# tomcreutz/slam-uwv_kalman_filters

Measured on AMD Instinct MI355X. Metric: UKF predict+update steps/sec at batch=65536 PoseUKF instances, 1 & 8 GPU, higher is better.
Workload: dtype f64

## Files before the change

### slam-uwv_kalman_filters_amd/csrc/uwvk_dev.hpp

```cpp
#pragma once
#include <hip/hip_runtime.h>
#include <stdint.h>

#include <cmath>

#define UWVK_DEV __device__ __forceinline__

namespace uwvk {

void clear_hip_error();
void note_hip_error(int err, const char* where);
inline int edevice_status(hipError_t e, const char* where) {
  note_hip_error((int)e, where);
  return 5;
}
inline int launch_sync_status(hipError_t launch, hipStream_t st, const char* where) {
  const hipError_t s = hipStreamSynchronize(st);
  if (launch != hipSuccess) return edevice_status(launch, where);
  if (s != hipSuccess) return edevice_status(s, where);
  return 0;
}
struct DeviceGuard {
  int prev = -1;
  explicit DeviceGuard(int device) {
// ... 58 lines not shown
}

UWVK_DEV void qmul(const double a[4], const double b[4], double o[4]) {
  double w = a[0] * b[0] - a[1] * b[1] - a[2] * b[2] - a[3] * b[3];
  double x = a[0] * b[1] + a[1] * b[0] + a[2] * b[3] - a[3] * b[2];
  double y = a[0] * b[2] + a[2] * b[0] + a[3] * b[1] - a[1] * b[3];
  double z = a[0] * b[3] + a[3] * b[0] + a[1] * b[2] - a[2] * b[1];
  o[0] = w; o[1] = x; o[2] = y; o[3] = z;
}

UWVK_DEV void qrot(const double q[4], const double v[3], double o[3]) {
  double uv[3], t[3];
  cross3(q + 1, v, uv);
  uv[0] += uv[0]; uv[1] += uv[1]; uv[2] += uv[2];
  cross3(q + 1, uv, t);
#pragma unroll
  for (int i = 0; i < 3; i++) o[i] = v[i] + q[0] * uv[i] + t[i];
}
UWVK_DEV void qrot_inv(const double q[4], const double v[3], double o[3]) {
  double c[4] = {q[0], -q[1], -q[2], -q[3]};
  qrot(c, v, o);
}
UWVK_DEV void qmatrix(const double q[4], double R[9]) {
  double w = q[0], x = q[1], y = q[2], z = q[3];
  double tx = 2 * x, ty = 2 * y, tz = 2 * z;
  double twx = tx * w, twy = ty * w, twz = tz * w;
  double txx = tx * x, txy = ty * x, txz = tz * x;
  double tyy = ty * y, tyz = tz * y, tzz = tz * z;
  R[0] = 1 - (tyy + tzz); R[1] = txy - twz; R[2] = txz + twy;
  R[3] = txy + twz; R[4] = 1 - (txx + tzz); R[5] = tyz - twx;
  R[6] = txz - twy; R[7] = tyz + twx; R[8] = 1 - (txx + tyy);
}

UWVK_DEV void so3_exp(const double v[3], double o[4]) {
  double t = sqrt(v[0] * v[0] + v[1] * v[1] + v[2] * v[2]);
  if (t == 0.0) { o[0] = 1; o[1] = o[2] = o[3] = 0; return; }
  double s, c;
  sincos(0.5 * t, &s, &c);
  s = s / t;
  o[0] = c; o[1] = s * v[0]; o[2] = s * v[1]; o[3] = s * v[2];
}
UWVK_DEV void so3_log(const double q[4], double o[3]) {
  double w = q[0], x = q[1], y = q[2], z = q[3];
  if (w < 0) { w = -w; x = -x; y = -y; z = -z; }
  double nv = sqrt(x * x + y * y + z * z);
  if (nv == 0.0) { o[0] = o[1] = o[2] = 0; return; }
  double k = 2.0 * atan2(nv, w) / nv;
  o[0] = k * x; o[1] = k * y; o[2] = k * z;
}
UWVK_DEV void qboxminus(const double a[4], const double b[4], double o[3]) {
  double bc[4] = {b[0], -b[1], -b[2], -b[3]}, r[4];
  qmul(a, bc, r);
  so3_log(r, o);
}

UWVK_DEV void qmul_side(const double a[4], const double b[4], double o[4], int swap) {
  const double sg = swap ? -1.0 : 1.0;
  const double cx = a[2] * b[3] - a[3] * b[2], cy = a[3] * b[1] - a[1] * b[3], cz = a[1] * b[2] - a[2] * b[1];
  o[0] = a[0] * b[0] - a[1] * b[1] - a[2] * b[2] - a[3] * b[3];
  o[1] = a[0] * b[1] + a[1] * b[0] + sg * cx;
  o[2] = a[0] * b[2] + a[2] * b[0] + sg * cy;
  o[3] = a[0] * b[3] + a[3] * b[0] + sg * cz;
}
UWVK_DEV void qplus_side(const double e[4], const double q[4], double o[4], int right) {
  if (!right) {
    qmul(e, q, o);
    return;
  }
  qmul_side(e, q, o, 1);
}
UWVK_DEV void qboxminus_side(const double a[4], const double b[4], double o[3], int right) {
  double bc[4] = {b[0], -b[1], -b[2], -b[3]}, r[4];
  if (!right) {
    qmul(a, bc, r);
  } else {
    qmul_side(a, bc, r, 1);
  }
  so3_log(r, o);
}

UWVK_DEV int lane_id() { return threadIdx.x & 63; }

UWVK_DEV int64_t xcd_instance(int64_t batch) {
  const int64_t w = blockIdx.x, n = batch >> 3;
  return w < (n << 3) ? (w & 7) * n + (w >> 3) : w;
}

UWVK_DEV constexpr int pidx(int i, int j) { return i >= j ? i * (i + 1) / 2 + j : j * (j + 1) / 2 + i; }
template <int DOF>
constexpr int tri_n() { return DOF * (DOF + 1) / 2; }

UWVK_DEV void unpack(int e, int& i, int& j) {
  int r = (int)((__builtin_sqrtf(8.0f * (float)e + 1.0f) - 1.0f) * 0.5f);
  if ((r + 1) * (r + 2) / 2 <= e) r++;
  if (r * (r + 1) / 2 > e) r--;
  i = r;
  j = e - r * (r + 1) / 2;
}

UWVK_DEV double shfl_d(double v, int src) {
  int lo = __double2loint(v), hi = __double2hiint(v);
  lo = __shfl(lo, src, 64);
  hi = __shfl(hi, src, 64);
  return __hiloint2double(hi, lo);
}
UWVK_DEV double readlane_d(double v, int lane) {
  int lo = __builtin_amdgcn_readlane(__double2loint(v), lane);
  int hi = __builtin_amdgcn_readlane(__double2hiint(v), lane);
  return __hiloint2double(hi, lo);
}
UWVK_DEV double shfl_xor_d(double v, int m) {
  int lo = __double2loint(v), hi = __double2hiint(v);
  lo = __shfl_xor(lo, m, 64);
  hi = __shfl_xor(hi, m, 64);
  return __hiloint2double(hi, lo);
}
UWVK_DEV double wave_sum(double v) {
#pragma unroll
  for (int m = 32; m >= 1; m >>= 1) v += shfl_xor_d(v, m);
  return v;
}

typedef double d4_t __attribute__((ext_vector_type(4)));

UWVK_DEV d4_t mfma_f64(double a, double b, d4_t c) { return __builtin_amdgcn_mfma_f64_16x16x4f64(a, b, c, 0, 0, 0); }

#ifdef UWVK_STAMPS
static __device__ unsigned long long uwvk_stamp_sum[64];
static __device__ unsigned long long uwvk_stamp_cnt[64];
UWVK_DEV unsigned long long stamp_now() {
  unsigned long long t;
  asm volatile("s_memtime %0\n\ts_waitcnt lgkmcnt(0)" : "=s"(t)::"memory");
  return t;
}
struct Stamper {
  unsigned long long last;
  UWVK_DEV Stamper() : last(stamp_now()) {}
  UWVK_DEV void mark(int ph) {
    __builtin_amdgcn_sched_barrier(0);
    const unsigned long long t = stamp_now();
    __builtin_amdgcn_sched_barrier(0);
    if (threadIdx.x == 0 && (blockIdx.x & 63) == 0) {
      atomicAdd(&uwvk_stamp_sum[ph], t - last);
      atomicAdd(&uwvk_stamp_cnt[ph], 1ull);
    }
    last = t;
  }
};
#else
struct Stamper {
  UWVK_DEV void mark(int) {}
};
#endif
#define UWVK_STAMP(ph) \
  do {                 \
    if (st) st->mark(ph); \
  } while (0)

}
```

### slam-uwv_kalman_filters_amd/csrc/uwvk_psp_dev.hpp

```cpp
#pragma once
#include <cstddef>

#include "uwvk_pose_dev.hpp"


#ifndef PSP_PAIR
#define PSP_PAIR 0
#endif
#ifndef PSP_NS
#define PSP_NS psp
#endif

namespace uwvk {
namespace PSP_NS {

constexpr int kLanes = PSP_PAIR ? 32 : 64;

UWVK_DEV void chain_prio_hi() { __builtin_amdgcn_s_setprio(1); }
UWVK_DEV void chain_prio_lo() { __builtin_amdgcn_s_setprio(0); }

template <int DOF>
struct PG {
  static constexpr int NP = DOF * (DOF + 1) / 2;
  static constexpr int NSLOT = (NP + kLanes - 1) / kLanes;
  static constexpr int N = 2 * DOF + 1;
  static constexpr int KP = 15;
  static constexpr int STG = 115;
};

template <int DOF>
struct alignas(16) PspSmem {
  double S[PG<DOF>::NP];
  double mu[Lay<DOF>::store];
  double stg[PG<DOF>::STG];
};
static_assert(sizeof(PspSmem<53>) <= 12800, "12 instances per CU");
static_assert(offsetof(PspSmem<53>, mu) == sizeof(double) * PG<53>::NP, "mu follows S");
static_assert(offsetof(PspSmem<53>, stg) == sizeof(double) * (PG<53>::NP + Lay<53>::store), "stg follows mu");
static_assert(offsetof(PspSmem<26>, mu) == sizeof(double) * PG<26>::NP, "mu follows S");
static_assert(offsetof(PspSmem<26>, stg) == sizeof(double) * (PG<26>::NP + Lay<26>::store), "stg follows mu");
constexpr int kPdLane0 = 27, kPdN = 27;
template <int DOF>
struct alignas(16) PspSmemPD : PspSmem<DOF> {
  double pS[32];
  double pm[32];
};
template <int DOF, int PD>
struct SmemT {
  using type = PspSmem<DOF>;
};
template <int DOF>
struct SmemT<DOF, 1> {
  using type = PspSmemPD<DOF>;
};
template <int DOF>
UWVK_DEV double* pd_ptr(PspSmem<DOF>&) {
  return nullptr;
}
template <int DOF>
UWVK_DEV double* pd_ptr(PspSmemPD<DOF>& s) {
  return s.pS;
}
UWVK_DEV constexpr int pd_dof(int d) { return d < 19 ? d : d + 27; }
UWVK_DEV constexpr int pd_store(int s) { return s < 20 ? s : s + 27; }

template <int DOF>
UWVK_DEV double* flat(PspSmem<DOF>& sm) {
  return reinterpret_cast<double*>(&sm);
}
template <int DOF>
UWVK_DEV const double* flat(const PspSmem<DOF>& sm) {
  return reinterpret_cast<const double*>(&sm);
}
template <int DOF>
constexpr int kFlatMu = PG<DOF>::NP;


UWVK_DEV int olane() {
  int l = PSP_PAIR ? ((int)threadIdx.x & 31) : (int)threadIdx.x;
  asm volatile("" : "+v"(l));
  return l;
}

template <class F>
UWVK_DEV constexpr unsigned long long lane_mask(F f) {
  unsigned long long m = 0;
  for (int i = 0; i < 64; i++)
    if (f(PSP_PAIR ? (i & 31) : i)) m |= 1ull << i;
  return m;
}
UWVK_DEV constexpr unsigned long long rep_mask(unsigned long long m) {
  return PSP_PAIR ? ((m & 0xFFFFFFFFull) | ((m & 0xFFFFFFFFull) << 32)) : m;
}
UWVK_DEV constexpr bool mask_needs_split(unsigned long long m) {
  return m >= 0xFFFFFFFF80000000ull && m < 0xFFFFFFFFFFFFFFF0ull;
}
UWVK_DEV bool lane_in_split(unsigned long long m) {
  unsigned lo = (unsigned)m, hi = (unsigned)(m >> 32);
  asm volatile("" : "+s"(lo), "+s"(hi));
  return __builtin_amdgcn_inverse_ballot_w64(((unsigned long long)hi << 32) | lo);
}
template <unsigned long long M>
UWVK_DEV bool lane_const() {
  if constexpr (mask_needs_split(M)) return lane_in_split(M);
  else return __builtin_amdgcn_inverse_ballot_w64(M);
}
#define LANE_IF(l, expr)                                                                                        \
  ({                                                                                                            \
    constexpr unsigned long long m_ = ::uwvk::PSP_NS::lane_mask([](int l) constexpr { return (bool)(expr); }); \
    ::uwvk::PSP_NS::lane_const<m_>();                                                                           \
  })
#define LANE_IN(m)                                                                     \
  (::uwvk::PSP_NS::mask_needs_split(::uwvk::PSP_NS::rep_mask(m))                       \
       ? ::uwvk::PSP_NS::lane_in_split(::uwvk::PSP_NS::rep_mask(m))                    \
       : __builtin_amdgcn_inverse_ballot_w64(::uwvk::PSP_NS::rep_mask(m)))
UWVK_DEV bool upper_half() { return lane_const<0xFFFFFFFF00000000ull>(); }
#if PSP_PAIR
template <int J>
UWVK_DEV double hbc(double v) {
  static_assert(J >= 0 && J < 16, "row_newbcast lane");
  int lo = __builtin_amdgcn_mov_dpp(__double2loint(v), 0x150 + J, 0xf, 0xf, false);
  int hi = __builtin_amdgcn_mov_dpp(__double2hiint(v), 0x150 + J, 0xf, 0xf, false);
  lo = __builtin_amdgcn_update_dpp(lo, lo, 0x142, 0xa, 0xf, false);
  hi = __builtin_amdgcn_update_dpp(hi, hi, 0x142, 0xa, 0xf, false);
  return __hiloint2double(hi, lo);
}
#endif
UWVK_DEV double hread(double v, int j) {
#if PSP_PAIR
  if (__builtin_constant_p(j) && j >= 0 && j < 16) {
    switch (j) {
      case 0: return hbc<0>(v);
      case 1: return hbc<1>(v);
      case 2: return hbc<2>(v);
      case 3: return hbc<3>(v);
      case 4: return hbc<4>(v);
      case 5: return hbc<5>(v);
      case 6: return hbc<6>(v);
      case 7: return hbc<7>(v);
      case 8: return hbc<8>(v);
      case 9: return hbc<9>(v);
      case 10: return hbc<10>(v);
      case 11: return hbc<11>(v);
      case 12: return hbc<12>(v);
      case 13: return hbc<13>(v);
      case 14: return hbc<14>(v);
      default: return hbc<15>(v);
    }
  }
  const double a = readlane_d(v, j), b = readlane_d(v, 32 + j);
  return upper_half() ? b : a;
#else
  return readlane_d(v, j);
#endif
}
UWVK_DEV int hlane(int j) { return PSP_PAIR ? j + ((int)threadIdx.x & 32) : j; }
// ... 54 lines not shown
#if PSP_PAIR
  static_assert(NL <= 32, "pair: one instance per 32-lane half");
  if constexpr (NL <= 16) return hread(s, 15);
  s = s + dpp_d<0x142, 0xa, 0xf>(s);
  return hread(s, 31);
#else
  if constexpr (NL <= 16) return readlane_d(s, 15);
  s = s + dpp_d<0x142, 0xa, 0xf>(s);
  if constexpr (NL <= 32) return readlane_d(s, 31);
  s = s + dpp_d<0x143, 0xc, 0xf>(s);
  return readlane_d(s, 63);
#endif
}
UWVK_DEV double sk(double c) {
  asm volatile("" : "+s"(c));
  return c;
}
UWVK_DEV void so3_exp_psp(const double v[3], double o[4]) {
  const double t2 = v[0] * v[0] + v[1] * v[1] + v[2] * v[2];
  if (t2 < 0.0625) {
    const double u = 0.25 * t2;
    double s = u * sk(-1.0 / 39916800.0);
    s = s + sk(1.0 / 362880.0);
    s = fma(s, u, sk(-1.0 / 5040.0));
    s = fma(s, u, sk(1.0 / 120.0));
    s = fma(s, u, sk(-1.0 / 6.0));
    s = fma(s, u, 1.0);
    s = 0.5 * s;
    double c = u * sk(-1.0 / 3628800.0);
    c = c + sk(1.0 / 40320.0);
    c = fma(c, u, sk(-1.0 / 720.0));
    c = fma(c, u, sk(1.0 / 24.0));
    c = fma(c, u, -0.5);
    c = fma(c, u, 1.0);
    o[0] = c; o[1] = s * v[0]; o[2] = s * v[1]; o[3] = s * v[2];
  } else {
    so3_exp(v, o);
  }
}
UWVK_DEV void so3_log_psp(const double q[4], double o[3]) {
  double w = q[0], x = q[1], y = q[2], z = q[3];
  if (w < 0) { w = -w; x = -x; y = -y; z = -z; }
  const double n2 = x * x + y * y + z * z, w2 = w * w;
  if (n2 < 0.0025 * w2) {
    double iw = __builtin_amdgcn_rcp(w);
    iw = fma(iw, fma(-w, iw, 1.0), iw);
    iw = fma(iw, fma(-w, iw, 1.0), iw);
    const double r2 = n2 * (iw * iw);
    double a = r2 * sk(-1.0 / 13.0);
    a = fma(a, -r2, sk(1.0 / 11.0));
    a = fma(a, -r2, sk(1.0 / 9.0));
    a = fma(a, -r2, sk(1.0 / 7.0));
    a = fma(a, -r2, sk(1.0 / 5.0));
    a = fma(a, -r2, sk(1.0 / 3.0));
    a = fma(a, -r2, 1.0);
    const double k = 2.0 * a * iw;
    o[0] = k * x; o[1] = k * y; o[2] = k * z;
  } else {
    so3_log(q, o);
  }
}
template <int SR>
UWVK_DEV void qplus_psp(const double e[4], const double q[4], double o[4]) {
  if constexpr (SR) qmul(q, e, o);
  else qmul(e, q, o);
}
template <int SR>
UWVK_DEV void qboxminus_psp(const double a[4], const double b[4], double o[3]) {
  double bc[4] = {b[0], -b[1], -b[2], -b[3]}, r[4];
  if constexpr (SR) qmul(bc, a, r);
  else qmul(a, bc, r);
  so3_log_psp(r, o);
}

UWVK_DEV double swap_pair_d(double v) { return dpp_d<0xb1, 0xf, 0xf>(v); }

UWVK_DEV double sel3(double v0, double v1, double v2, int i) { return i == 0 ? v0 : (i == 1 ? v1 : v2); }
UWVK_DEV double sel6(double v0, double v1, double v2, double v3, double v4, double v5, int i) {
  return i < 3 ? sel3(v0, v1, v2, i) : sel3(v3, v4, v5, i - 3);
}

UWVK_DEV int pidx_sel(int p, int j, int Tj) { return j >= p ? Tj + p : p * (p + 1) / 2 + j; }
UWVK_DEV int pidx_sel_b(int p, int j, int Tj, bool ge) { return ge ? Tj + p : p * (p + 1) / 2 + j; }

UWVK_DEV void wsync() {
  __builtin_amdgcn_fence(__ATOMIC_RELEASE, "wavefront");
  __builtin_amdgcn_wave_barrier();
  __builtin_amdgcn_fence(__ATOMIC_ACQUIRE, "wavefront");
}

template <int R, int NL, int STRIDE>
UWVK_DEV void lds_sums(const double (&v)[R], double* buf, int l, double (&out)[R]) {
  static_assert(NL % 2 == 0 && R * NL <= 115, "transpose buffer (PG::STG)");
  const int c = l / STRIDE;
  if (l % STRIDE == 0 && c < NL) {
#pragma unroll
    for (int i = 0; i < R; i++) buf[i * NL + c] = v[i];
  }
  wsync();
  const double* row = buf + (l < R ? l : 0) * NL;
  double p[NL / 2];
#pragma unroll
  for (int k = 0; k < NL / 2; k++) p[k] = row[2 * k] + row[2 * k + 1];
#pragma unroll
  for (int w = 1; w < NL / 2; w *= 2)
#pragma unroll
    for (int k = 0; k + w < NL / 2; k += 2 * w) p[k] += p[k + w];
#pragma unroll
  for (int i = 0; i < R; i++) out[i] = hread(p[0], i);
}

#define PSP_PHASE(ph) \
  do {                \
    UWVK_STAMP(ph);   \
    l = olane();      \
  } while (0)

UWVK_DEV void psync() {
  __builtin_amdgcn_fence(__ATOMIC_RELEASE, "workgroup");
  __builtin_amdgcn_s_barrier();
  __builtin_amdgcn_fence(__ATOMIC_ACQUIRE, "workgroup");
}

UWVK_DEV constexpr bool scaled_dof(int d) { return d >= 12 && d != 18; }

template <int K, int J>
UWVK_DEV void pchol_step_lds(double (&a)[K], int r, bool& ok, double* col, double* rows, int q, double piv,
                             double inv_in, double& chk) {
  if constexpr (J < K) {
    ok = ok && (piv > 0.0);
    const double inv = rsqrt_f64(piv);
    a[J] = LANE_IF(r, r >= J) ? a[J] * inv : 0.0;
    double pnext = 0.0, invn = 0.0;
    if constexpr (J + 1 < K) {
      pnext = hread(a[J + 1] - a[J] * a[J], J + 1);
    }
    if constexpr (J + 1 < K) {
      constexpr int C0 = J + 1;
      double* const cj = col + (((C0 & 1) == 0) ? 1 : 0);
      static_assert(64 + 1 <= 115, "column slots (PG::STG)");
      cj[r & 63] = a[J];
      __builtin_amdgcn_fence(__ATOMIC_RELEASE, "wavefront");
      __builtin_amdgcn_wave_barrier();
      __builtin_amdgcn_fence(__ATOMIC_ACQUIRE, "wavefront");
#pragma unroll
      for (int c = C0; c < K; c++) a[c] -= a[J] * cj[c];
#pragma unroll
      for (int c = J + 1; c < K; c++) asm volatile("" : "+v"(a[c]));
    }
    pchol_step_lds<K, J + 1>(a, r, ok, col, rows, q, pnext, invn, chk);
  }
}

constexpr int STG_ROWS = 0;

template <int DOF, int K, class RL>
UWVK_DEV bool pchol(const double* S, int r, double (&a)[K], double dl, double* stg) {
  const int rr = r < DOF ? r : DOF - 1;
  const double* Sr = S + rr * (rr + 1) / 2;
#pragma unroll
  for (int c = 0; c < K; c++) a[c] = Sr[c] * (scaled_dof(c) ? dl * hread(dl, c) : dl);
  bool ok = true;
  static_assert(rows_ascending<RL>(), "RL::rows ascending");
  constexpr unsigned long long rm = rep_mask(rows_mask<RL>());
  int q = (int)__builtin_amdgcn_mbcnt_hi((unsigned)(rm >> 32), __builtin_amdgcn_mbcnt_lo((unsigned)rm, 0u));
  if constexpr (PSP_PAIR) q -= upper_half() ? __builtin_popcount((unsigned)rm) : 0;
  static_assert(RL::NR >= 1 && STG_ROWS + RL::NR * K <= 115, "staging area (PG::STG)");
  const double p0 = hread(a[0], 0);
  const double inv0 = rsqrt_f64(p0);
  double chk = fma(inv0, 0.0, 0.0);
  pchol_step_lds<K, 0>(a, r, ok, stg + STG_ROWS, stg + STG_ROWS, q, p0, inv0, chk);
  if (LANE_IN(rows_mask<RL>())) {
    double* rp = stg + STG_ROWS + q * K;
#pragma unroll
    for (int J = 0; J < K; J++) rp[J] = a[J];
  }
  psync();
  return ok;
}

template <int NR>
UWVK_DEV constexpr int row_pos(const int (&rows)[NR], int d) {
  for (int q = 0; q < NR; q++)
    if (rows[q] == d) return q;
  return -1;
}

template <class RL, int DOF, int K, int Q>
UWVK_DEV void gen_rows_q(const double* mu, const double* stg, int j, double sg, double (&v)[3], double* x) {
  if constexpr (Q < RL::NR) {
    constexpr int d = RL::rows[Q];
    const double l = stg[Q * K + j];
    if constexpr (d >= 3 && d < 6) {
      v[d - 3] = sg * l;
    } else {
      x[d2s(d)] = mu[d2s(d)] + sg * l;
    }
    gen_rows_q<RL, DOF, K, Q + 1>(mu, stg, j, sg, v, x);
  }
}
template <class RL>
UWVK_DEV constexpr bool has_rot() {
  for (int q = 0; q < RL::NR; q++)
    if (RL::rows[q] >= 3 && RL::rows[q] < 6) return true;
  return false;
}
template <class RL, int DOF, int K, int SR>
UWVK_DEV void gen_rows(const double* mu, const double* stg, int p, double x[Lay<DOF>::store]) {
  using L = Lay<DOF>;
#pragma unroll
  for (int s = 0; s < L::store; s++) x[s] = mu[s];
  if constexpr (K > 0) {
    const bool in = LANE_IF(p, p < 2 * K);
    const int j = in ? (p >> 1) : 0;
    const double sg = in ? (LANE_IF(p, (p & 1) != 0) ? -1.0 : 1.0) : 0.0;
    double v[3] = {0.0, 0.0, 0.0};
    gen_rows_q<RL, DOF, K, 0>(mu, stg, j, sg, v, x);
    if constexpr (has_rot<RL>()) {
      double e[4];
      so3_exp_psp(v, e);
      qplus_psp<SR>(e, mu + L::s_quat, x + L::s_quat);
    }
  }
}

template <int DOF, int SR>
UWVK_DEV void proc_orientation(const double x[Lay<DOF>::store], const PoseShared& sh, const ProcCtx& c, double o[4]) {
  using L = Lay<DOF>;
  const double dl = x[L::s_pos] * sh.inv_rm;
  double sl, cl;
  if (fabs(dl) < 0.01) {
    const double u = dl * dl;
    double sd = fma(fma(fma(u * sk(1.0 / 362880.0) + sk(-1.0 / 5040.0), u, sk(1.0 / 120.0)), u, sk(-1.0 / 6.0)), u, 1.0) * dl;
    double cd = fma(fma(fma(u * sk(1.0 / 40320.0) + sk(-1.0 / 720.0), u, sk(1.0 / 24.0)), u, -0.5), u, 1.0);
    sl = sh.slat0 * cd + sh.clat0 * sd;
    cl = sh.clat0 * cd - sh.slat0 * sd;
  } else {
    sincos(sh.lat0 + dl, &sl, &cl);
  }
  const double er[3] = {kEarthW * cl, 0.0, kEarthW * sl};
  double wb[3], wn[3];
#pragma unroll
  for (int i = 0; i < 3; i++) wb[i] = c.w[i] - x[L::s_bg + i];
  qrot(x + L::s_quat, wb, wn);
#pragma unroll
  for (int i = 0; i < 3; i++) wn[i] = (wn[i] - er[i]) * c.dt;
  double e[4];
  so3_exp_psp(wn, e);
  qplus_psp<SR>(e, x + L::s_quat, o);
}

UWVK_DEV double proc_vect_lane(int s, const double* mu, const ProcCtx& c) {
  const double x = mu[s];
  const double y = mu[c.vpart >= 0 ? c.vpart : s];
  const double d = c.vpart >= 0 ? y : c.nt_lane * (x - c.off_lane);
  return (c.vpart >= 0 || c.nt_lane != 0.0) ? x + c.dt * d : x;
}

template <int DOF>
UWVK_DEV double tan_ntau_sel(int d, const PoseShared& sh) {
  using L = Lay<DOF>;
  double nt = 0.0;
  nt = (d >= L::d_bg && d < L::d_bg + 3) ? sh.ntau[0] : nt;
  nt = (d >= L::d_ba && d < L::d_ba + 3) ? sh.ntau[1] : nt;
  if constexpr (L::has_params) {
    nt = (d >= L::d_inertia && d < L::d_inertia + 9) ? sh.ntau[2] : nt;
    nt = (d >= L::d_lin && d < L::d_lin + 9) ? sh.ntau[3] : nt;
    nt = (d >= L::d_quad && d < L::d_quad + 9) ? sh.ntau[4] : nt;
  }
  nt = (d >= L::d_wv && d < L::d_wv + 4) ? sh.ntau[5] : nt;
  nt = (d >= L::d_badcp && d < L::d_badcp + 2) ? sh.ntau[6] : nt;
  nt = (d == L::d_rho) ? sh.ntau[7] : nt;
  return nt;
}
UWVK_DEV constexpr int proc_couple(int d) { return d < 3 ? d + 6 : (d >= 6 && d < 9 ? d + 3 : -1); }

struct PredRows {
  static constexpr int NR = 7;
  static constexpr int rows[NR] = {0, 3, 4, 5, 12, 13, 14};
};

struct LaneQ {
  double q0, q1, q2;
};
template <int DOF, int PD = 0>
UWVK_DEV LaneQ lane_q(const double* fq, int l) {
  const double2* f2 = reinterpret_cast<const double2*>(fq);
  LaneQ q{0.0, 0.0, 0.0};
  if (l < DOF) {
    q.q0 = f2[pidx(l, l)].y;
    if (l >= 1) q.q1 = f2[pidx(l, l - 1)].y;
    if (l >= 2) q.q2 = f2[pidx(l, l - 2)].y;
  }
  if constexpr (PD && !PSP_PAIR) {
    if (l >= kPdLane0 && l < kPdLane0 + kPdN) q.q0 = f2[PG<DOF>::NP + (l - kPdLane0)].y;
  }
  return q;
}

template <int DOF, int QM = 0, int SR = 0, int PD = 0>
UWVK_DEV bool psp_predict(PspSmem<DOF>& sm, const PoseShared& sh, const ProcCtx& pc, const double* Q,
                          const double* fq, double& ds, double& ids, const LaneQ& lq,
                          Stamper* st = nullptr, double* px = nullptr) {
  using L = Lay<DOF>;
  using G = PG<DOF>;
  constexpr int K = G::KP;
  static_assert(!PD || (DOF == 26 && QM == 1), "PD: the 26-DOF layout, lane-resident Q");
  constexpr int NW = PD ? 53 : DOF;
  int l = olane();
  const double dt = pc.dt, dt2 = dt * dt;
  double qo_lane = 0.0;
  if (LANE_IF(l, l < 9)) {
    double R[9];
    qmatrix(sm.mu + L::s_quat, R);
    const int r = l / 3, c = l % 3;
    double Rr[3], Rc[3];
#pragma unroll
    for (int m = 0; m < 3; m++) {
      Rr[m] = sel3(R[m], R[3 + m], R[6 + m], r);
      Rc[m] = sel3(R[m], R[3 + m], R[6 + m], c);
    }
    double s = 0.0;
#pragma unroll
    for (int k = 0; k < 3; k++) {
// ... 397 lines not shown
        H[r][7 + i] = r == i ? 1.0 : 0.0;
      }
    }
  }
};
template <int DOF>
struct PXY {
  static constexpr int M = 2, K = 0, NR = 2, NC = 2, ZMODE = 0, GATE = 0;
  static constexpr int rows[NR] = {0, 1};
  static constexpr int cols[NC] = {0, 1};
  int gate = 0;
  UWVK_DEV void eval(const double* x, double (&z)[M]) const { z[0] = x[0]; z[1] = x[1]; }
  UWVK_DEV void jac(const double*, double (&H)[M][NC]) const { H[0][0] = 1; H[0][1] = 0; H[1][0] = 0; H[1][1] = 1; }
};
template <int DOF>
struct PZ {
  static constexpr int M = 1, K = 0, NR = 1, NC = 1, ZMODE = 0, GATE = 0;
  static constexpr int rows[NR] = {2};
  static constexpr int cols[NC] = {2};
  UWVK_DEV void eval(const double* x, double (&z)[M]) const { z[0] = x[2]; }
  UWVK_DEV void jac(const double*, double (&H)[M][NC]) const { H[0][0] = 1; }
};

template <int DOF>
struct PEffVO {
  static constexpr int M = 6, K = 9, NR = 3, NC = 0, ZMODE = 0, GATE = 0;
  static constexpr int rows[NR] = {6, 7, 8};
  static constexpr int cols[1] = {6};
  HConstrain<DOF> h;
  UWVK_DEV void eval(const double* x, double (&z)[M]) const { h(x, z); }
  UWVK_DEV void jac(const double*, double (&)[M][1]) const {}
};

template <int R, int NL, int STRIDE, int C0 = 0>
UWVK_DEV void lds_sums_chunked(const double (&v)[R], double* buf, int l, double (&out)[R]) {
  if constexpr (C0 < R) {
    constexpr int CH0 = 115 / NL, CH = (R - C0) < CH0 ? (R - C0) : CH0;
    double vc[CH], oc[CH];
#pragma unroll
    for (int i = 0; i < CH; i++) vc[i] = v[C0 + i];
    lds_sums<CH, NL, STRIDE>(vc, buf, l, oc);
#pragma unroll
    for (int i = 0; i < CH; i++) out[C0 + i] = oc[i];
    wsync();
    lds_sums_chunked<R, NL, STRIDE, C0 + CH>(v, buf, l, out);
  }
}

#if !PSP_PAIR
template <int DOF, int I, int NT>
UWVK_DEV void rankm_block(double* S, const double (&Aop)[NT], const double (&Bop)[NT], int q, int c, int tq) {
  if constexpr (I < NT) {
    constexpr int O = DOF - 16 * NT;
    int base[4];
#pragma unroll
    for (int i = 0; i < 4; i++) {
      const int x = O + 16 * I + 4 * i;
      base[i] = q * x + (x * (x + 1) / 2) + tq;
    }
    d4_t acc[I + 1];
    using LdsV = const volatile __attribute__((address_space(3))) double*;
    LdsV rp[4];
#pragma unroll
    for (int i = 0; i < 4; i++) {
      rp[i] = (LdsV)(S + base[i]);
      asm volatile("" : "+v"(rp[i]));
    }
#pragma unroll
    for (int J = 0; J <= I; J++)
#pragma unroll
      for (int i = 0; i < 4; i++) acc[J][i] = rp[i][16 * J];
#pragma unroll
    for (int J = 0; J <= I; J++) acc[J] = mfma_f64(Aop[I], Bop[J], acc[J]);
    if constexpr (I == 0) asm volatile("" : "+v"(acc[0]));
    else if constexpr (I == 1) asm volatile("" : "+v"(acc[0]), "+v"(acc[1]));
    else if constexpr (I == 2) asm volatile("" : "+v"(acc[0]), "+v"(acc[1]), "+v"(acc[2]));
    else asm volatile("" : "+v"(acc[0]), "+v"(acc[1]), "+v"(acc[2]), "+v"(acc[3]));
    constexpr unsigned long long diagm[4] = {
        lane_mask([](int l) constexpr { return (l & 15) <= ((l >> 4) & 3) + 0; }),
        lane_mask([](int l) constexpr { return (l & 15) <= ((l >> 4) & 3) + 4; }),
        lane_mask([](int l) constexpr { return (l & 15) <= ((l >> 4) & 3) + 8; }),
        lane_mask([](int l) constexpr { return (l & 15) <= ((l >> 4) & 3) + 12; })};
    using LdsW = __attribute__((address_space(3))) double*;
#pragma unroll
    for (int J = 0; J <= I; J++)
#pragma unroll
      for (int i = 0; i < 4; i++)
        if (J < I || LANE_IN(diagm[i])) ((LdsW)rp[i])[16 * J] = acc[J][i];
    rankm_block<DOF, I + 1, NT>(S, Aop, Bop, q, c, tq);
  }
}

template <int DOF, int M>
UWVK_DEV void rankm_mfma_o(double* S, double* stg, const double (&Ct)[M], const double (&Kt)[M], int l) {
  static_assert(M <= 3, "rank <= 3 (K = 4 with zero padding)");
  constexpr int NT = DOF / 16, O = DOF - 16 * NT;
  static_assert(NT >= 1 && NT <= 4, "frame");
  static_assert(2 * 16 * M <= PG<DOF>::STG, "operand blocks (PG::STG)");
  constexpr bool kStripLds = 2 * 16 * M + O * M <= PG<DOF>::STG;
  const int q = (l >> 4) & 3, c = l & 15;
  double Aop[NT], Bop[NT];
#pragma unroll
  for (int T = 0; T < NT; T++) {
    const int src = l - O - 16 * T;
    if (src >= 0 && src < 16) {
#pragma unroll
      for (int k = 0; k < M; k++) {
        stg[src * M + k] = Ct[k];
        stg[16 * M + src * M + k] = Kt[k];
      }
    }
    if (kStripLds && T == 0 && LANE_IF(l, l < O)) {
#pragma unroll
      for (int k = 0; k < M; k++) stg[32 * M + l * M + k] = Kt[k];
    }
    wsync();
    const int qq = LANE_IF(l, ((l >> 4) & 3) < M) ? q : 0;
    const double a = stg[c * M + qq], b = stg[16 * M + c * M + qq];
    Aop[T] = LANE_IF(l, ((l >> 4) & 3) < M) ? -a : 0.0;
    Bop[T] = LANE_IF(l, ((l >> 4) & 3) < M) ? b : 0.0;
    wsync();
  }
  if constexpr (O > 0) {
    double kc[O][M];
#pragma unroll
    for (int j = 0; j < O; j++)
#pragma unroll
      for (int k = 0; k < M; k++) kc[j][k] = kStripLds ? stg[32 * M + j * M + k] : readlane_d(Kt[k], j);
    {
      const int lc = l < DOF ? l : DOF - 1;
      const int b0 = (lc * (lc + 1)) >> 1;
      double sv[O];
#pragma unroll
      for (int j = 0; j < O; j++) sv[j] = S[b0 + (j <= lc ? j : lc)];
      double nv[O];
#pragma unroll
      for (int j = O - 1; j >= 0; j--) {
        double s2 = sv[j];
#pragma unroll
        for (int k = 0; k < M; k++) s2 = fma(-Ct[k], kc[j][k], s2);
        nv[j] = s2;
      }
      if (l < DOF) {
#pragma unroll
        for (int j = O - 1; j >= 0; j--) S[b0 + (j <= lc ? j : lc)] = nv[j];
      }
    }
  }
  rankm_block<DOF, 0, NT>(S, Aop, Bop, q, c, ((q * (q + 1)) >> 1) + O + c);
}

#else
template <int DOF>
UWVK_DEV constexpr unsigned long long rankm_col_mask(int j) {
  unsigned long long m = 0;
  for (int l = 0; l < 64; l++)
    if (l >= j && l < DOF) m |= 1ull << l;
  return m;
}
template <int DOF, int M>
UWVK_DEV void rankm_rows(double* S, double* stg, const double (&Ct)[M], const double (&Kt)[M], int l) {
  static_assert(DOF * M <= PG<DOF>::STG, "K~ rows (PG::STG)");
  constexpr int RB = 4;
  if (l < DOF) {
#pragma unroll
    for (int k = 0; k < M; k++) stg[l * M + k] = Kt[k];
  }
  wsync();
  const int lc = l < DOF ? l : DOF - 1;
  const int b0 = (lc * (lc + 1)) >> 1;
#pragma unroll
  for (int j0 = 0; j0 < DOF; j0 += RB) {
    double sv[RB];
#pragma unroll
    for (int u = 0; u < RB; u++)
      if (j0 + u < DOF) sv[u] = S[b0 + j0 + u];
#pragma unroll
    for (int u = 0; u < RB; u++) {
      if (j0 + u >= DOF) continue;
      double s2 = sv[u];
#pragma unroll
      for (int k = 0; k < M; k++) s2 = fma(-Ct[k], stg[(j0 + u) * M + k], s2);
      if (LANE_IN(rankm_col_mask<DOF>(j0 + u))) S[b0 + j0 + u] = s2;
    }
  }
  wsync();
}
#endif

UWVK_DEV double hfma(double h, double x, double acc) {
  if (__builtin_constant_p(h) && h == 0.0) return acc;
  return acc + h * x;
}

template <int DOF, int SR>
UWVK_DEV void psp_apply_delta(PspSmem<DOF>& sm, double dl, int l) {
  using L = Lay<DOF>;
  const double dv[3] = {hread(dl, 3), hread(dl, 4), hread(dl, 5)};
  double R[9], eq[4];
  so3_exp_psp(dv, eq);
  {
    const double tq[4] = {eq[0], SR ? -eq[1] : eq[1], SR ? -eq[2] : eq[2], SR ? -eq[3] : eq[3]};
    qmatrix(tq, R);
  }
  double nb;
  {
    const int lc = l < DOF ? l : DOF - 1;
    const int Tl = (lc * (lc + 1)) >> 1;
    const int e0 = pidx_sel_b(3, lc, Tl, LANE_IN(col_ge_mask<DOF>(3, false))),
              e1 = pidx_sel_b(4, lc, Tl, LANE_IN(col_ge_mask<DOF>(4, false))),
              e2 = pidx_sel_b(5, lc, Tl, LANE_IN(col_ge_mask<DOF>(5, false)));
    double s0 = sm.S[e0], s1 = sm.S[e1], s2 = sm.S[e2];
    asm volatile("" : "+v"(s0), "+v"(s1), "+v"(s2));
    double B[9];
#pragma unroll
    for (int u = 0; u < 3; u++)
#pragma unroll
      for (int v = 0; v < 3; v++) B[u * 3 + v] = sm.S[pidx(3 + u, 3 + v)];
    const int r = l / 3, c = l % 3;
    double sb = 0.0;
#pragma unroll
    for (int u = 0; u < 3; u++) {
      double t = 0.0;
#pragma unroll
      for (int v = 0; v < 3; v++) t += B[u * 3 + v] * sel3(R[v], R[3 + v], R[6 + v], c);
      sb += sel3(R[u], R[3 + u], R[6 + u], r) * t;
    }
    nb = sb;
    double n3[3];
#pragma unroll
    for (int i = 0; i < 3; i++) n3[i] = R[i * 3] * s0 + R[i * 3 + 1] * s1 + R[i * 3 + 2] * s2;
    if (LANE_IF(l, l < DOF && !(l >= 3 && l < 6))) {
      sm.S[e0] = n3[0];
      sm.S[e1] = n3[1];
      sm.S[e2] = n3[2];
    }
  }
  const double dsh = dpp_d<0x138, 0xf, 0xf>(dl);
  double mnew = flat(sm)[kFlatMu<DOF> + (l & 63)] + 1.0 * (LANE_IF(l, l < 3) ? dl : dsh);
  asm volatile("" : "+v"(mnew));
  double qn[4];
  qplus_psp<SR>(eq, sm.mu + L::s_quat, qn);
  psync();
  if (LANE_IF(l, l < 9 && (l / 3) >= (l % 3))) sm.S[pidx(3 + l / 3, 3 + l % 3)] = nb;
  if (LANE_IF(l, l < L::store && !(l >= 3 && l < 7))) sm.mu[l] = mnew;
  if (LANE_IF(l, l < 4)) sm.mu[3 + l] = qn[l];
  psync();
}

template <int DOF, int SR, class HM, int NW = DOF>
UWVK_DEV bool psp_update(PspSmem<DOF>& sm, const double (&z)[HM::M], const double (&Rm)[HM::M * HM::M], int gate,
                         const HM& hm, bool* ok, double ds, double ids, Stamper* st = nullptr) {
  using L = Lay<DOF>;
  constexpr int M = HM::M, K = HM::K, NC = HM::NC, KA = K > 0 ? K : 1, NCA = NC > 0 ? NC : 1;
  static_assert(!PSP_PAIR || 2 * K + 1 <= 32, "pair: the 2k + 1 sigma points of an update fit 32 lanes");
  int l = olane();
  double a[KA];
  bool cok = true;
  if constexpr (K > 0) {
    chain_prio_hi();
    cok = pchol<DOF, K, HM>(sm.S, l, a, ds, sm.stg);
    chain_prio_lo();
  }
  PSP_PHASE(30);
  [[maybe_unused]] const bool pt = LANE_IF(l, l < 2 * K);
  double zp[M];
  {
    double x[L::store];
    gen_rows<HM, DOF, K, SR>(sm.mu, sm.stg + STG_ROWS, l, x);
    hm.eval(x, zp);
  }
  double zc[M], zb[M], e[M];
#pragma unroll
  for (int i = 0; i < M; i++) zc[i] = hread(zp[i], 2 * K);
  constexpr double wc = 1.0 + 2.0 * (NW - K);
  double S[M * M];
  double Hs[M][NCA];
  hm.jac(sm.mu, Hs);
  double Pl = 0.0;
  if constexpr (K > 0) {
    const int q = LANE_IF(l, l < M * K) ? l : 0;
    const int i = q / K, j = q - (q / K) * K;
    double lv[NCA];
#pragma unroll
    for (int t = 0; t < NC; t++) lv[t] = sm.stg[STG_ROWS + row_pos(HM::rows, HM::cols[t]) * K + j];
#pragma unroll
    for (int ii = 0; ii < M; ii++) {
      double pr = 0.0;
#pragma unroll
      for (int t = 0; t < NC; t++) pr = hfma(Hs[ii][t], lv[t], pr);
      Pl = (ii == 0 || i == ii) ? pr : Pl;
    }
    constexpr int R = M + M * (M + 1) / 2;
    double v[R], sums[R];
#pragma unroll
    for (int i2 = 0; i2 < M; i2++) v[i2] = zp[i2] - zc[i2];
    int k = M;
#pragma unroll
    for (int i2 = 0; i2 < M; i2++)
#pragma unroll
      for (int j2 = 0; j2 <= i2; j2++) v[k++] = v[i2] * v[j2];
    if constexpr (R * 2 * K <= 115) lds_sums<R, 2 * K, 1>(v, sm.stg, l, sums);
    else lds_sums_chunked<R, 2 * K, 1>(v, sm.stg, l, sums);
    double m[M];
#pragma unroll
    for (int i2 = 0; i2 < M; i2++) {
      m[i2] = sums[i2] * (1.0 / (double)(2 * NW + 1));
      zb[i2] = zc[i2] + m[i2];
      e[i2] = zc[i2] - zb[i2];
    }
    k = M;
#pragma unroll
    for (int i2 = 0; i2 < M; i2++)
#pragma unroll
      for (int j2 = 0; j2 <= i2; j2++) {
        const double s = sums[k++] - m[i2] * sums[j2] - m[j2] * sums[i2] + (2.0 * K) * m[i2] * m[j2];
        S[i2 * M + j2] = 0.5 * (s + wc * e[i2] * e[j2]);
      }
  } else {
#pragma unroll
    for (int i2 = 0; i2 < M; i2++) {
      zb[i2] = zc[i2];
      e[i2] = 0.0;
#pragma unroll
      for (int j2 = 0; j2 <= i2; j2++) S[i2 * M + j2] = 0.0;
    }
  }
  double zd[M];
#pragma unroll
  for (int i = 0; i < M; i++) zd[i] = K > 0 ? zp[i] - swap_pair_d(zp[i]) : 0.0;
  PSP_PHASE(31);
  const int rl = l < DOF ? l : DOF - 1;
  const int Trl = (rl * (rl + 1)) >> 1;
  double Gr[M];
#pragma unroll
  for (int i = 0; i < M; i++) Gr[i] = 0.0;
#pragma unroll
  for (int t = 0; t < NC; t++) {
    double s = sm.S[pidx_sel_b(HM::cols[t], rl, Trl, LANE_IN(col_ge_mask<DOF>(HM::cols[t], false)))];
    if (scaled_dof(HM::cols[t])) s = s * hread(ds, HM::cols[t]);
#pragma unroll
    for (int i = 0; i < M; i++) Gr[i] = hfma(Hs[i][t], s, Gr[i]);
  }
#pragma unroll
  for (int i = 0; i < M; i++) Gr[i] = Gr[i] * ds;
  PSP_PHASE(32);
  double Gl[M], C[M];
  if constexpr (K > 0) {
    constexpr int PS = M == 3 ? 4 : M, P0 = M >= 2 ? 1 : 0;
    static_assert(P0 + 2 * PS * K <= PG<DOF>::STG, "P and Dz (PG::STG)");
    if (LANE_IF(l, l < M * K)) sm.stg[P0 + (l % K) * PS + l / K] = Pl;
    if (LANE_IF(l, (l & 1) == 0 && l < 2 * K)) {
#pragma unroll
      for (int i = 0; i < M; i++) sm.stg[P0 + PS * K + (l >> 1) * PS + i] = zd[i];
    }
    wsync();
    double g[M], c[M];
#pragma unroll
    for (int i = 0; i < M; i++) {
      g[i] = Gr[i];
      c[i] = 0.0;
    }
#pragma unroll
    for (int j = 0; j < K; j++) {
      double pj[M], zj[M];
#pragma unroll
      for (int i = 0; i < M; i++) {
        pj[i] = sm.stg[P0 + j * PS + i];
        zj[i] = sm.stg[P0 + PS * K + j * PS + i];
      }
#pragma unroll
      for (int i = 0; i < M; i++) {
        g[i] -= a[j] * pj[i];
        c[i] += a[j] * zj[i];
        asm volatile("" : "+v"(g[i]), "+v"(c[i])::"memory");
      }
    }
    wsync();
#pragma unroll
    for (int i = 0; i < M; i++) {
      Gl[i] = g[i];
      C[i] = g[i] + 0.5 * c[i];
    }
  } else {
#pragma unroll
    for (int i = 0; i < M; i++) {
      Gl[i] = Gr[i];
      C[i] = Gr[i];
    }
  }
#if PSP_PAIR
  double glb[NCA][M];
  {
    static_assert(NC * M <= PG<DOF>::STG, "Gl staging (PG::STG)");
    constexpr unsigned long long cm = cols_mask<HM>();
    static_assert(NC == 0 || (cm != 0 && (cm >> 32) == 0), "HM::cols ascending, below 32");
    const int t = (int)__builtin_amdgcn_mbcnt_hi((unsigned)(rep_mask(cm) >> 32),
                                                  __builtin_amdgcn_mbcnt_lo((unsigned)rep_mask(cm), 0u)) -
                  (upper_half() ? __builtin_popcount((unsigned)cm) : 0);
    if (LANE_IN(cm)) {
#pragma unroll
      for (int j = 0; j < M; j++) sm.stg[t * M + j] = Gl[j];
    }
    wsync();
#pragma unroll
    for (int tt = 0; tt < NC; tt++)
#pragma unroll
      for (int j = 0; j < M; j++) glb[tt][j] = sm.stg[tt * M + j];
    wsync();
  }
#endif
#pragma unroll
  for (int i = 0; i < M; i++)
#pragma unroll
    for (int j = 0; j <= i; j++) {
      double hg = 0.0;
#pragma unroll
#if PSP_PAIR
      for (int t = 0; t < NC; t++) hg = hfma(Hs[i][t], glb[t][j], hg);
#else
      for (int t = 0; t < NC; t++) hg = hfma(Hs[i][t], hread(Gl[j], HM::cols[t]), hg);
#endif
      const double s = S[i * M + j] + hg;
      S[i * M + j] = s + Rm[i * M + j];
      if (j != i) S[j * M + i] = s + Rm[j * M + i];
    }
  double Si[M * M];
  small_inv<M>(S, Si);
  double Kg[M];
#pragma unroll
  for (int i = 0; i < M; i++) {
    double s = 0.0;
#pragma unroll
    for (int j = 0; j < M; j++) s += C[j] * Si[j * M + i];
    Kg[i] = s;
  }
  double nu[M];
#pragma unroll
  for (int i = 0; i < M; i++) nu[i] = z[i] - zb[i];
  double d2 = 0.0;
#pragma unroll
  for (int j = 0; j < M; j++) {
    double u = 0.0;
#pragma unroll
    for (int i = 0; i < M; i++) u += nu[i] * Si[i * M + j];
    d2 += u * nu[j];
  }
  *ok = cok;
  const bool accept = gate == 0 ? true : !(d2 > kD2P95);
  if (!accept) return false;
  PSP_PHASE(33);
  psync();
  double dl = 0.0;
#pragma unroll
  for (int i = 0; i < M; i++) dl += Kg[i] * nu[i];
  double Ct[M], Kt[M];
#pragma unroll
  for (int i = 0; i < M; i++) {
    Ct[i] = C[i] * ids;
    Kt[i] = Kg[i] * ids;
  }
  psync();
#if PSP_PAIR
  rankm_rows<DOF, M>(sm.S, sm.stg, Ct, Kt, l);
#else
  if constexpr (M <= 3) {
    rankm_mfma_o<DOF, M>(sm.S, sm.stg, Ct, Kt, l);
  } else {
    double c0[3], k0[3], c1[M - 3], k1[M - 3];
#pragma unroll
    for (int i = 0; i < 3; i++) { c0[i] = Ct[i]; k0[i] = Kt[i]; }
#pragma unroll
    for (int i = 0; i < M - 3; i++) { c1[i] = Ct[3 + i]; k1[i] = Kt[3 + i]; }
    rankm_mfma_o<DOF, 3>(sm.S, sm.stg, c0, k0, l);
    psync();
    rankm_mfma_o<DOF, M - 3>(sm.S, sm.stg, c1, k1, l);
  }
#endif
  psync();
  PSP_PHASE(34);
  psp_apply_delta<DOF, SR>(sm, dl, l);
  PSP_PHASE(35);
  return true;
}


#if !PSP_PAIR
template <int DOF, int P, int W>
UWVK_DEV void eff_chol_update(double* S, int l) {
  constexpr int NRT = (DOF - P + 15) / 16, NS = P / 4;
  const int q = (l >> 4) & 3, c = l & 15;
  const int bc = P + c < DOF ? P + c : DOF - 1;
  const double* Bp = S + ((bc * (bc + 1)) >> 1);
  const bool bv = c < W;
  double Bop[NS];
#pragma unroll
  for (int s = 0; s < NS; s++) Bop[s] = bv ? Bp[4 * s + q] : 0.0;
#pragma unroll
  for (int t = 0; t < NRT; t++) {
    const int ar = P + 16 * t + c;
    const int arc = ar < DOF ? ar : DOF - 1;
    const double* Ap = S + ((arc * (arc + 1)) >> 1);
    const bool av = ar < DOF;
    int idx[4];
    bool st[4];
    d4_t acc;
#pragma unroll
    for (int i = 0; i < 4; i++) {
      const int row = P + 16 * t + q + 4 * i, col = P + c;
      st[i] = row < DOF && bv && col <= row;
      const int rr = row < DOF ? row : DOF - 1;
      const int cc = col <= rr ? col : rr;
      idx[i] = ((rr * (rr + 1)) >> 1) + cc;
      acc[i] = S[idx[i]];
    }
#pragma unroll
    for (int s = 0; s < NS; s++) acc = mfma_f64(av ? -Ap[4 * s + q] : 0.0, Bop[s], acc);
#pragma unroll
    for (int i = 0; i < 4; i++)
      if (st[i]) S[idx[i]] = acc[i];
  }
}

template <int P, int W, int J>
UWVK_DEV void eff_chol_step(double (&a)[W], int r, bool& ok, double* col) {
  if constexpr (J < W) {
    const double piv = readlane_d(a[J], P + J);
    ok = ok && (piv > 0.0);
    const double inv = rsqrt_f64(piv);
    a[J] = LANE_IF(r, r >= P + J) ? a[J] * inv : 0.0;
    if constexpr (J + 1 < W) {
      col[r & 63] = a[J];
      wsync();
#pragma unroll
      for (int c = J + 1; c < W; c++) a[c] -= a[J] * col[P + c];
#pragma unroll
      for (int c = J + 1; c < W; c++) asm volatile("" : "+v"(a[c]));
    }
    eff_chol_step<P, W, J + 1>(a, r, ok, col);
  }
}

struct PanelMasks {
  unsigned long long m[16];
};
template <int P, int W, int LIM>
UWVK_DEV constexpr PanelMasks panel_masks() {
  PanelMasks g{};
  for (int c = 0; c < W; c++) {
    unsigned long long m = 0;
    for (int i = 0; i < 64; i++)
      if (i >= P + c && i < LIM) m |= 1ull << i;
    g.m[c] = m;
  }
  return g;
}

template <int DOF, int P>
UWVK_DEV void eff_chol(double* S, double* col, int l, bool& ok) {
  if constexpr (P < DOF) {
    constexpr int W = DOF - P < 16 ? DOF - P : 16;
    if constexpr (P > 0) {
      eff_chol_update<DOF, P, W>(S, l);
      psync();
    }
    const int rr = l < DOF ? l : DOF - 1;
    double* Sr = S + ((rr * (rr + 1)) >> 1) + P;
    constexpr PanelMasks ld = panel_masks<P, W, 64>(), stm = panel_masks<P, W, DOF>();
    double a[W];
#pragma unroll
    for (int c = 0; c < W; c++) {
      const double v = Sr[c];
      a[c] = LANE_IN(ld.m[c]) ? v : 0.0;
    }
    eff_chol_step<P, W, 0>(a, l, ok, col);
#pragma unroll
    for (int c = 0; c < W; c++)
      if (LANE_IN(stm.m[c])) Sr[c] = a[c];
    psync();
    eff_chol<DOF, P + 16>(S, col, l, ok);
  }
}

template <int DOF, int SR>
UWVK_DEV void eff_point_quat(const PspSmem<DOF>& sm, int j, double sg, double (&q)[4]) {
  using L = Lay<DOF>;
  double v[3];
#pragma unroll
  for (int d = 3; d < 6; d++) {
    const bool in = j <= d;
    const double ld = sm.S[d * (d + 1) / 2 + (in ? j : d)];
    v[d - 3] = sg * (in ? ld : 0.0);
  }
  double e[4];
  so3_exp_psp(v, e);
  qplus_psp<SR>(e, sm.mu + L::s_quat, q);
}
template <int DOF, int K, class HM>
UWVK_DEV void eff_point(const PspSmem<DOF>& sm, const HM& h, int j, double sg, const double (&q)[4],
                        double (&z)[6]) {
  using L = Lay<DOF>;
  double x[L::store];
#pragma unroll
  for (int s = 0; s < L::store; s++) x[s] = sm.mu[s];
#pragma unroll
  for (int i = 0; i < 4; i++) x[L::s_quat + i] = q[i];
#pragma unroll
  for (int d = 0; d < K; d++) {
    if (d >= 3 && d < 6) continue;
    const bool in = j <= d;
    const double ld = sm.S[d * (d + 1) / 2 + (in ? j : d)];
    x[d2s(d)] = sm.mu[d2s(d)] + sg * (in ? ld : 0.0);
  }
  h(x, z);
}

template <int R, int NL, int CAP, int C0 = 0>
// ... 206 lines not shown
```

Measured before the change: 402.4 million.

## Tile rank-M covariance downdate into 4x4 register blocks and pair Cholesky columns

In the PSP_PAIR path, the row-per-lane rank-M update of the packed covariance is replaced by a scheme where each lane owns one 4x4 tile of the lower triangle. C and K operands are staged through LDS once per tile, so each lane reuses its loaded operands across 16 entries instead of re-reading stg for every element. The partial Cholesky now eliminates two columns per step, sharing one LDS exchange per pair instead of one per column. A compile-time phase-marker macro is also added for profiling. This adds LDS round trips and masked store groups, and it only takes effect when PSP_PAIR is enabled.

```diff
diff --git a/slam-uwv_kalman_filters_amd/csrc/uwvk_dev.hpp b/slam-uwv_kalman_filters_amd/csrc/uwvk_dev.hpp
--- a/slam-uwv_kalman_filters_amd/csrc/uwvk_dev.hpp
+++ b/slam-uwv_kalman_filters_amd/csrc/uwvk_dev.hpp
@@ -234,9 +234,19 @@
   UWVK_DEV void mark(int) {}
 };
 #endif
+#ifdef UWVK_PHASE_MARKS
+#define UWVK_STAMP(ph)                           \
+  do {                                           \
+    (void)st;                                    \
+    __builtin_amdgcn_sched_barrier(0);           \
+    asm volatile("; uwvk_phase %0" ::"n"(ph));   \
+    __builtin_amdgcn_sched_barrier(0);           \
+  } while (0)
+#else
 #define UWVK_STAMP(ph) \
   do {                 \
     if (st) st->mark(ph); \
   } while (0)
-
-}
+#endif
+
+}
diff --git a/slam-uwv_kalman_filters_amd/csrc/uwvk_psp_dev.hpp b/slam-uwv_kalman_filters_amd/csrc/uwvk_psp_dev.hpp
--- a/slam-uwv_kalman_filters_amd/csrc/uwvk_psp_dev.hpp
+++ b/slam-uwv_kalman_filters_amd/csrc/uwvk_psp_dev.hpp
@@ -2,6 +2,7 @@
 #include <cstddef>
 
 #include "uwvk_pose_dev.hpp"
+#include "uwvk_tiles.hpp"
 
 
 #ifndef PSP_PAIR
@@ -362,14 +363,69 @@
   }
 }
 
+#if PSP_PAIR
+template <int K, int J>
+UWVK_DEV void pchol_step2_lds(double (&a)[K], const double (&f)[K], int r, bool& ok, double* col2, double piv) {
+#pragma clang fp contract(off)
+  if constexpr (J + 1 == K) {
+    ok = ok && (piv > 0.0);
+    const double inv = rsqrt_f64(piv);
+    a[J] = LANE_IF(r, r >= J) ? a[J] * inv : 0.0;
+  } else if constexpr (J + 1 < K) {
+    static_assert(J + 1 < 16, "hbc lanes");
+    ok = ok && (piv > 0.0);
+    const double inv0 = rsqrt_f64(piv);
+    a[J] = LANE_IF(r, r >= J) ? a[J] * inv0 : 0.0;
+    a[J + 1] = fma(-a[J], hread(a[J], J + 1), a[J + 1]);
+    const double piv1 = hread(a[J + 1], J + 1);
+    ok = ok && (piv1 > 0.0);
+    const double inv1 = rsqrt_f64(piv1);
+    a[J + 1] = LANE_IF(r, r >= J + 1) ? a[J + 1] * inv1 : 0.0;
+    double pnext = 0.0;
+    if constexpr (J + 2 < K) {
+      {
+        const double t = J == 0 ? fma(f[J + 2], a[J + 2], -(a[J] * a[J])) : fma(-a[J], a[J], a[J + 2]);
+        pnext = hread(fma(-a[J + 1], a[J + 1], t), J + 2);
+      }
+      static_assert(2 * kLanes + 1 <= 115, "column pair slots (PG::STG)");
+      double* const c2 = static_cast<double*>(__builtin_assume_aligned(col2, 16));
+      double* const w = static_cast<double*>(__builtin_assume_aligned(c2 + 2 * (r & (kLanes - 1)), 16));
+      w[0] = a[J];
+      w[1] = a[J + 1];
+      __builtin_amdgcn_fence(__ATOMIC_RELEASE, "wavefront");
+      __builtin_amdgcn_wave_barrier();
+      __builtin_amdgcn_fence(__ATOMIC_ACQUIRE, "wavefront");
+#pragma unroll
+      for (int c = J + 2; c < K; c++) {
+        const double t = J == 0 ? fma(f[c], a[c], -(a[J] * c2[2 * c])) : fma(-a[J], c2[2 * c], a[c]);
+        a[c] = fma(-a[J + 1], c2[2 * c + 1], t);
+      }
+#pragma unroll
+      for (int c = J + 2; c < K; c++) asm volatile("" : "+v"(a[c]));
+    }
+    pchol_step2_lds<K, J + 2>(a, f, r, ok, col2, pnext);
+  }
+}
+#endif
+
 constexpr int STG_ROWS = 0;
 
 template <int DOF, int K, class RL>
 UWVK_DEV bool pchol(const double* S, int r, double (&a)[K], double dl, double* stg) {
   const int rr = r < DOF ? r : DOF - 1;
   const double* Sr = S + rr * (rr + 1) / 2;
+#if PSP_PAIR
+  static_assert(K >= 2, "column pairs");
+  double f[K];
+#pragma unroll
+  for (int c = 0; c < K; c++) {
+    f[c] = scaled_dof(c) ? dl * hread(dl, c) : dl;
+    a[c] = c < 2 ? Sr[c] * f[c] : Sr[c];
+  }
+#else
 #pragma unroll
   for (int c = 0; c < K; c++) a[c] = Sr[c] * (scaled_dof(c) ? dl * hread(dl, c) : dl);
+#endif
   bool ok = true;
   static_assert(rows_ascending<RL>(), "RL::rows ascending");
   constexpr unsigned long long rm = rep_mask(rows_mask<RL>());
@@ -377,9 +433,13 @@
   if constexpr (PSP_PAIR) q -= upper_half() ? __builtin_popcount((unsigned)rm) : 0;
   static_assert(RL::NR >= 1 && STG_ROWS + RL::NR * K <= 115, "staging area (PG::STG)");
   const double p0 = hread(a[0], 0);
+#if PSP_PAIR
+  pchol_step2_lds<K, 0>(a, f, r, ok, stg + ((PG<DOF>::NP + Lay<DOF>::store) & 1), p0);
+#else
   const double inv0 = rsqrt_f64(p0);
   double chk = fma(inv0, 0.0, 0.0);
   pchol_step_lds<K, 0>(a, r, ok, stg + STG_ROWS, stg + STG_ROWS, q, p0, inv0, chk);
+#endif
   if (LANE_IN(rows_mask<RL>())) {
     double* rp = stg + STG_ROWS + q * K;
 #pragma unroll
@@ -1083,36 +1143,86 @@
 
 #else
 template <int DOF>
-UWVK_DEV constexpr unsigned long long rankm_col_mask(int j) {
-  unsigned long long m = 0;
-  for (int l = 0; l < 64; l++)
-    if (l >= j && l < DOF) m |= 1ull << l;
-  return m;
+struct TileStoreGroups {
+  unsigned long long m[16];
+  bool lead[16];
+  unsigned long long rbm[3], cbm[3];
+};
+template <int DOF>
+UWVK_DEV constexpr TileStoreGroups<DOF> tile_store_groups() {
+  TileStoreGroups<DOF> g{};
+  for (int p = 0; p < 16; p++) {
+    g.m[p] = tiles::store_mask(DOF, p / 4, p % 4);
+    g.lead[p] = g.m[p] != 0;
+    for (int q = 0; q < p; q++)
+      if (g.m[q] == g.m[p]) g.lead[p] = false;
+  }
+  for (int b = 0; b < 3; b++) {
+    g.rbm[b] = tiles::block_bit_mask(DOF, false, b);
+    g.cbm[b] = tiles::block_bit_mask(DOF, true, b);
+  }
+  return g;
 }
 template <int DOF, int M>
-UWVK_DEV void rankm_rows(double* S, double* stg, const double (&Ct)[M], const double (&Kt)[M], int l) {
-  static_assert(DOF * M <= PG<DOF>::STG, "K~ rows (PG::STG)");
-  constexpr int RB = 4;
-  if (l < DOF) {
-#pragma unroll
-    for (int k = 0; k < M; k++) stg[l * M + k] = Kt[k];
-  }
+UWVK_DEV void rankm_tiles(PspSmem<DOF>& sm, const double (&Ct)[M], const double (&Kt)[M], int l) {
+  constexpr int TB = tiles::TB;
+  static_assert(TB == 4 && tiles::num_tiles(DOF) <= kLanes && tiles::block_bits(DOF) <= 3, "one 4x4 tile per local lane");
+  constexpr int ST0 = (PG<DOF>::NP + Lay<DOF>::store) & 1;
+  static_assert(ST0 + kLanes * M <= PG<DOF>::STG, "one operand's slots (PG::STG)");
+  static_assert((TB * M) % 2 == 0, "a tile's operands start aligned");
+  static_assert(tiles::max_load_index(DOF) < (int)(sizeof(PspSmem<DOF>) / sizeof(double)),
+                "tile loads past the triangle stay in PspSmem");
+  constexpr TileStoreGroups<DOF> G = tile_store_groups<DOF>();
+  double* const st = sm.stg + ST0;
+  double* const fl = flat(sm);
+  int rb = 0, cb = 0;
+#pragma unroll
+  for (int b = 0; b < 3; b++) {
+    if (G.rbm[b]) rb |= LANE_IN(G.rbm[b]) ? (1 << b) : 0;
+    if (G.cbm[b]) cb |= LANE_IN(G.cbm[b]) ? (1 << b) : 0;
+  }
+#pragma unroll
+  for (int k = 0; k < M; k++) st[l * M + k] = Kt[k];
   wsync();
-  const int lc = l < DOF ? l : DOF - 1;
-  const int b0 = (lc * (lc + 1)) >> 1;
-#pragma unroll
-  for (int j0 = 0; j0 < DOF; j0 += RB) {
-    double sv[RB];
-#pragma unroll
-    for (int u = 0; u < RB; u++)
-      if (j0 + u < DOF) sv[u] = S[b0 + j0 + u];
-#pragma unroll
-    for (int u = 0; u < RB; u++) {
-      if (j0 + u >= DOF) continue;
-      double s2 = sv[u];
-#pragma unroll
-      for (int k = 0; k < M; k++) s2 = fma(-Ct[k], stg[(j0 + u) * M + k], s2);
-      if (LANE_IN(rankm_col_mask<DOF>(j0 + u))) S[b0 + j0 + u] = s2;
+  double kt[TB][M], ct[TB][M];
+  {
+    const double* kp = static_cast<const double*>(__builtin_assume_aligned(st + cb * (TB * M), 16));
+#pragma unroll
+    for (int v = 0; v < TB; v++)
+#pragma unroll
+      for (int k = 0; k < M; k++) kt[v][k] = kp[v * M + k];
+  }
+  const int i0 = TB * rb;
+  const int e0 = ((i0 * (i0 + 1)) >> 1) + TB * cb;
+  double sv[TB][TB];
+#pragma unroll
+  for (int u = 0; u < TB; u++)
+#pragma unroll
+    for (int v = 0; v < TB; v++) sv[u][v] = fl[e0 + u * i0 + tiles::tri(u) + v];
+  wsync();
+#pragma unroll
+  for (int k = 0; k < M; k++) st[l * M + k] = Ct[k];
+  wsync();
+  {
+    const double* cp = static_cast<const double*>(__builtin_assume_aligned(st + rb * (TB * M), 16));
+#pragma unroll
+    for (int u = 0; u < TB; u++)
+#pragma unroll
+      for (int k = 0; k < M; k++) ct[u][k] = cp[u * M + k];
+  }
+#pragma unroll
+  for (int u = 0; u < TB; u++)
+#pragma unroll
+    for (int v = 0; v < TB; v++)
+#pragma unroll
+      for (int k = 0; k < M; k++) sv[u][v] = fma(-ct[u][k], kt[v][k], sv[u][v]);
+#pragma unroll
+  for (int p = 0; p < 16; p++) {
+    if (!G.lead[p]) continue;
+    if (LANE_IN(G.m[p])) {
+#pragma unroll
+      for (int q = p; q < 16; q++)
+        if (G.m[q] == G.m[p]) fl[e0 + (q / 4) * i0 + tiles::tri(q / 4) + q % 4] = sv[q / 4][q % 4];
     }
   }
   wsync();
@@ -1393,7 +1503,7 @@
   }
   psync();
 #if PSP_PAIR
-  rankm_rows<DOF, M>(sm.S, sm.stg, Ct, Kt, l);
+  rankm_tiles<DOF, M>(sm, Ct, Kt, l);
 #else
   if constexpr (M <= 3) {
     rankm_mfma_o<DOF, M>(sm.S, sm.stg, Ct, Kt, l);
diff --git a/slam-uwv_kalman_filters_amd/csrc/uwvk_tiles.hpp b/slam-uwv_kalman_filters_amd/csrc/uwvk_tiles.hpp
--- /dev/null
+++ b/slam-uwv_kalman_filters_amd/csrc/uwvk_tiles.hpp
@@ -0,0 +1,56 @@
+#pragma once
+#include <cstdint>
+
+namespace uwvk {
+namespace tiles {
+
+constexpr int TB = 4;
+
+constexpr int tri(int n) { return n * (n + 1) / 2; }
+constexpr int row_blocks(int dof) { return (dof + TB - 1) / TB; }
+constexpr int num_tiles(int dof) { return tri(row_blocks(dof)); }
+
+constexpr int tile_rb(int t) {
+  int rb = 0;
+  while (tri(rb + 1) <= t) rb++;
+  return rb;
+}
+constexpr int tile_cb(int t) { return t - tri(tile_rb(t)); }
+
+constexpr int lane_tile(int dof, int l) { return l < num_tiles(dof) ? l : 0; }
+constexpr int lane_rb(int dof, int l) { return tile_rb(lane_tile(dof, l)); }
+constexpr int lane_cb(int dof, int l) { return tile_cb(lane_tile(dof, l)); }
+
+constexpr int entry_index(int dof, int l, int u, int v) {
+  return tri(TB * lane_rb(dof, l) + u) + TB * lane_cb(dof, l) + v;
+}
+constexpr int max_load_index(int dof) {
+  int m = 0;
+  for (int l = 0; l < 32; l++)
+    if (entry_index(dof, l, TB - 1, TB - 1) > m) m = entry_index(dof, l, TB - 1, TB - 1);
+  return m;
+}
+
+constexpr bool stores(int dof, int l, int u, int v) {
+  return l < num_tiles(dof) && TB * tile_rb(l) + u < dof && TB * tile_cb(l) + v <= TB * tile_rb(l) + u;
+}
+constexpr uint64_t store_mask(int dof, int u, int v) {
+  uint64_t m = 0;
+  for (int l = 0; l < 32; l++)
+    if (stores(dof, l, u, v)) m |= uint64_t(1) << l;
+  return m;
+}
+constexpr uint64_t block_bit_mask(int dof, bool col, int b) {
+  uint64_t m = 0;
+  for (int l = 0; l < 32; l++)
+    if (((col ? lane_cb(dof, l) : lane_rb(dof, l)) >> b) & 1) m |= uint64_t(1) << l;
+  return m;
+}
+constexpr int block_bits(int dof) {
+  int n = 0;
+  while ((1 << n) < row_blocks(dof)) n++;
+  return n;
+}
+
+}
+}
```

Measured after the change: 435.8 million, median of 6. +8.3%, better.
